# therealadityashankar/hey-buddy

Measured on AMD Instinct MI355X. Metric: audio clips/sec featurized+trained, 1.5 s @16 kHz, 1/2/4/8 GPU, higher is better.
Workload: dtype f32

## Files before the change

### hey-buddy_amd/csrc/hbk_augment.hip

```cpp
#include <algorithm>
#include <cmath>
#include <numeric>
#include <type_traits>
#include <vector>

#include "hbk_common.h"

namespace hbk {
namespace {

constexpr int kT = 23040;
constexpr int kM = kT / 2;
constexpr int kThreads = 1024;
constexpr int kN1 = 16000;
constexpr int kM1 = kN1 / 2;

template <bool INV>
__device__ __forceinline__ cf tw_const(double frac) {
  const double a = (INV ? 2.0 : -2.0) * M_PI * frac;
  return cf{static_cast<float>(cos(a)), static_cast<float>(sin(a))};
}

template <bool INV>
__device__ __forceinline__ void dft3(cf& a, cf& b, cf& c) {
// ... 1244 lines not shown
    tin[lc][32 + 4 * lq + 3] = p1.w;
    __syncthreads();
    const int tn = min(t0 + kEqTile, kT - kEqTile);
    p0 = *reinterpret_cast<const float4*>(xl + tn + 4 * lq);
    p1 = *reinterpret_cast<const float4*>(xl + tn + 32 + 4 * lq);
    for (int st0 = 0; st0 < kEqTile; st0 += 8) {
      const float4 ia = *reinterpret_cast<const float4*>(&tin[c][st0]);
      const float4 ib = *reinterpret_cast<const float4*>(&tin[c][st0 + 4]);
      const float in8[8] = {ia.x, ia.y, ia.z, ia.w, ib.x, ib.y, ib.z, ib.w};
      float o8[8];
#pragma unroll
      for (int q = 0; q < 8; ++q) {
        const float u = sec == 0 ? in8[q] : prev;
        const double vd = u;
        const double y = fma(b0, vd, s1);
        s1 = fma(b1, vd, fma(-a1, y, s2));
        s2 = fma(b2, vd, -a2 * y);
        const float v = static_cast<float>(y);
        o8[q] = v;
        prev = __builtin_bit_cast(float, __builtin_amdgcn_update_dpp(__builtin_bit_cast(int, prev),
                                                                     __builtin_bit_cast(int, v), 0x111, 0xF, 0xF,
                                                                     false));
      }
      if (sec == 6) {
        *reinterpret_cast<float4*>(&tout[c][st0]) = float4{o8[0], o8[1], o8[2], o8[3]};
        *reinterpret_cast<float4*>(&tout[c][st0 + 4]) = float4{o8[4], o8[5], o8[6], o8[7]};
      }
    }
    __syncthreads();
    if (store_l) {
#pragma unroll
      for (int m = 0; m < 8; ++m) {
        const int kk = lq + 8 * m;
        const int n = t0 - 6 + kk;
        if (n >= 0 && n < kT) ol[n] = tout[lc][kk];
      }
    }
    __syncthreads();
  }
}

constexpr int kPsFft = 250, kPsHop = 7, kPsBins = kPsFft / 2 + 1, kPsPad = kPsFft / 2;
constexpr int kPsTapMax = HBK_PITCH_SHIFT_MAX_TAPS;
constexpr int kPsPhaseMax = 128;
constexpr int kPsResFrames = 32;
#ifndef HBK_PV_ABLATE
#define HBK_PV_ABLATE 0
#endif
#ifndef HBK_PV_CLIPS
#define HBK_PV_CLIPS 2
#endif
constexpr int kPvClips = HBK_PV_CLIPS;
constexpr int kPvGroup = 8;
constexpr int kPvRows = 64;
constexpr int kPvGh = 64;
#ifndef HBK_PV_F32STATE
#define HBK_PV_F32STATE 0
#endif
#ifndef HBK_PV_RESTART
#if HBK_PV_F32STATE
#define HBK_PV_RESTART 128
#else
#define HBK_PV_RESTART 1024
#endif
#endif
constexpr int kPvRestart = HBK_PV_RESTART;
#if HBK_PV_F32STATE
typedef float pv_t;
#else
typedef double pv_t;
#endif

struct PitchArgs {
  const float* x;
  int64_t x_stride;
  const int32_t* idx;
  int n;
  float* out;
  int64_t out_stride;
  int L, f_in, f_out, l1, orig, nw, width, target;
  double rate;
  float* y;
  float* taps;
};

__device__ __forceinline__ int ps_i0(const PitchArgs& a, int t, float& alpha) {
  const float ts = static_cast<float>(static_cast<double>(t) * a.rate);
  const float fl = floorf(ts);
  alpha = ts - fl;
  return static_cast<int>(fl);
}

struct PvClip {
  float d[kPvRows][8];
  float xs[256];
  float gh[2][kPvGh][8];
  int cnt0;
};
struct PvShared {
  cf tw[256];
  double tw64[256][2];
  float4 wt[3][128];
  PvClip c[kPvClips];
};

__device__ __forceinline__ int pv_g(int b) { return (b & 3) ^ ((b & 4) ? 7 : 0); }

template <int kCtrl>
__device__ __forceinline__ float pv_dpp(float v) {
  return __builtin_bit_cast(float, __builtin_amdgcn_update_dpp(0, __builtin_bit_cast(int, v), kCtrl, 0xF, 0xF, true));
}

template <bool kSwap16>
__device__ __forceinline__ float pv_swap_add(float x, float y) {
  if (kSwap16)
    asm volatile("s_nop 1\n\tv_permlane16_swap_b32 %0, %1\n\ts_nop 1" : "+v"(x), "+v"(y));
  else
    asm volatile("s_nop 1\n\tv_permlane32_swap_b32 %0, %1\n\ts_nop 1" : "+v"(x), "+v"(y));
  return x + y;
}

__device__ __forceinline__ cf pv_cmul(cf a, cf b) {
  cf t, r;
  asm("v_pk_mul_f32 %0, %1, %2 op_sel_hi:[0,1]" : "=v"(t) : "v"(a), "v"(b));
  asm("v_pk_fma_f32 %0, %1, %2, %3 op_sel:[1,1,0] op_sel_hi:[1,0,1] neg_lo:[0,1,0]" : "=v"(r) : "v"(a), "v"(b), "v"(t));
  return r;
}
__device__ __forceinline__ cf pv_cmul_conj(cf a, cf b) {
  cf t, r;
  asm("v_pk_mul_f32 %0, %1, %2 op_sel_hi:[0,1] neg_hi:[0,1]" : "=v"(t) : "v"(a), "v"(b));
  asm("v_pk_fma_f32 %0, %1, %2, %3 op_sel:[1,1,0] op_sel_hi:[1,0,1]" : "=v"(r) : "v"(a), "v"(b), "v"(t));
  return r;
}

typedef float pv_v4 __attribute__((ext_vector_type(4)));
typedef __attribute__((address_space(3))) const pv_v4 pv_lds_v4;
__device__ __forceinline__ float4 pv_f4(pv_v4 v) { return float4{v.x, v.y, v.z, v.w}; }

__device__ __forceinline__ cf pv_inc(float4 da, float4 db, float4 w12, float4 w34, float4 w56) {
  const cf dxy = {da.x, da.y}, dzw = {da.z, da.w}, exy = {db.x, db.y}, ez = {db.z, db.w};
  const cf w1 = {w12.x, w12.y}, w2 = {w12.z, w12.w}, w3 = {w34.x, w34.y}, w4 = {w34.z, w34.w};
  const cf w5 = {w56.x, w56.y}, w6 = {w56.z, w56.w};
  cf acc;
  asm("v_pk_mul_f32 %0, %1, %2 op_sel:[1,0] op_sel_hi:[1,1]" : "=v"(acc) : "v"(dxy), "v"(w1));
  asm("v_pk_fma_f32 %0, %1, %2, %0 op_sel:[0,0,0] op_sel_hi:[0,1,1]" : "+v"(acc) : "v"(dzw), "v"(w2));
  asm("v_pk_fma_f32 %0, %1, %2, %0 op_sel:[1,0,0] op_sel_hi:[1,1,1]" : "+v"(acc) : "v"(dzw), "v"(w3));
  asm("v_pk_fma_f32 %0, %1, %2, %0 op_sel:[0,0,0] op_sel_hi:[0,1,1]" : "+v"(acc) : "v"(exy), "v"(w4));
  asm("v_pk_fma_f32 %0, %1, %2, %0 op_sel:[1,0,0] op_sel_hi:[1,1,1]" : "+v"(acc) : "v"(exy), "v"(w5));
  asm("v_pk_fma_f32 %0, %1, %2, %0 op_sel:[0,0,0] op_sel_hi:[0,1,1]" : "+v"(acc) : "v"(ez), "v"(w6));
  return acc;
}

__device__ __forceinline__ float ps_xp(const float* xr, int L, int p) {
  int i = p - kPsPad;
  i = i < 0 ? -i : i;
  i = i >= L ? 2 * (L - 1) - i : i;
  return xr[i];
}

__device__ __forceinline__ void pv_load_rows(const PitchArgs& a, PvShared& sh, const float* xr, int cl, int lane,
                                             int fb) {
  for (int q = lane; q < 2 * kPvRows; q += 128) {
    const int row = q >> 1, h = q & 1, f = fb + row;
    float* dr = sh.c[cl].d[row];
    if (f >= a.f_in) {
      for (int j = 4 * h; j < 4 * h + 4; ++j) dr[j] = 0.f;
      continue;
    }
    if (h == 0) {
      for (int j = 0; j < 4; ++j) dr[j] = ps_xp(xr, a.L, 7 * f + 243 + j) - ps_xp(xr, a.L, 7 * f - 7 + j);
    } else {
      int delta = 0;
      for (int j = 0; j < 7; ++j) {
        const float vin = ps_xp(xr, a.L, 7 * f + 243 + j), vout = ps_xp(xr, a.L, 7 * f - 7 + j);
        delta += (vin != 0.f) - (vout != 0.f);
        if (j >= 4) dr[j] = vin - vout;
      }
      dr[7] = __builtin_bit_cast(float, delta);
    }
  }
}

#ifdef HBK_PHASE_TIMING
#define HBK_PVT(i)                                     \
  do {                                                 \
    const unsigned long long t_ = __builtin_amdgcn_s_memtime(); \
    pvt[i] += t_ - pvt_t0;                             \
    pvt_t0 = t_;                                       \
  } while (0)
#else
#define HBK_PVT(i) \
  do {             \
  } while (0)
#endif

#ifndef HBK_PV_UNROLL_TAIL
#define HBK_PV_UNROLL_TAIL 1
#endif
#ifndef HBK_PV_WAVES
#define HBK_PV_WAVES 4
#endif
__global__ void __launch_bounds__(128 * kPvClips) __attribute__((amdgpu_waves_per_eu(HBK_PV_WAVES)))
ps_vocoder_kernel(PitchArgs a) {
#ifdef HBK_PHASE_TIMING
  unsigned long long pvt[5] = {0, 0, 0, 0, 0}, pvt_t0 = __builtin_amdgcn_s_memtime();
#endif
  extern __shared__ __attribute__((aligned(16))) unsigned char pv_smem[];
  PvShared& sh = *reinterpret_cast<PvShared*>(pv_smem);
  const int tid = threadIdx.x, cl = tid >> 7, lane = tid & 127;
  const int e = min(static_cast<int>(blockIdx.x) * kPvClips + cl, a.n - 1);
  const bool live = static_cast<int>(blockIdx.x) * kPvClips + cl < a.n;
  const float* xr = a.x + static_cast<int64_t>(a.idx[e]) * a.x_stride;
  PvClip& C = sh.c[cl];
  for (int q = tid; q < 256; q += blockDim.x) {
    double sn, cs;
    sincospi(2.0 * q / kPsFft, &sn, &cs);
    sh.tw[q] = cf{static_cast<float>(cs), static_cast<float>(sn)};
    sh.tw64[q][0] = cs;
    sh.tw64[q][1] = -sn;
  }
  if (lane == 0) C.cnt0 = 0;
  __syncthreads();
  int nz = 0;
  for (int q = lane; q < kPsFft; q += 128) {
    const float v = ps_xp(xr, a.L, q);
    C.xs[q] = v;
    nz += v != 0.f;
  }
  if (nz) atomicAdd(&C.cnt0, nz);
  for (int q = tid; q < 3 * 128; q += blockDim.x) {
    const int j = 2 * (q / 128) + 1, kk = min(q % 128, kPsBins - 1), q1 = (kk * j) % kPsFft,
              q2 = (kk * (j + 1)) % kPsFft;
    sh.wt[q / 128][q % 128] = float4{static_cast<float>(sh.tw64[q1][0]), static_cast<float>(sh.tw64[q1][1]),
                                     static_cast<float>(sh.tw64[q2][0]), static_cast<float>(sh.tw64[q2][1])};
  }
  int fb = 1;
  pv_load_rows(a, sh, xr, cl, lane, fb);
  __syncthreads();

  const int k = min(lane, kPsBins - 1);
  const int q7 = (7 * k) % kPsFft;
  const pv_t rr = static_cast<pv_t>(sh.tw64[q7][0]), ri = static_cast<pv_t>(-sh.tw64[q7][1]);
  const float ck = lane < kPsBins ? ((lane == 0 || lane == kPsBins - 1) ? 1.f : 2.f) : 0.f;
  const int gb = pv_g(lane & 7), w = lane >> 6, ou = (lane >> 3) & 7;
  cf esr[4], esi[4];
#pragma unroll
  for (int r = 0; r < 8; ++r) {
    const int sr = r ^ gb;
    const cf ev = sr < kPsHop ? ck * sh.tw[(k * sr) % kPsFft] : cf{0.f, 0.f};
    esr[r >> 1][r & 1] = ev.x;
    esi[r >> 1][r & 1] = -ev.y;
  }
  const bool b3 = lane & 8;
  auto direct = [&](double& re, double& im) {
    re = im = 0.0;
    int q = 0;
    for (int n = 0; n < kPsFft; ++n) {
      const double v = static_cast<double>(C.xs[n]);
      re = fma(v, sh.tw64[q][0], re);
      im = fma(v, sh.tw64[q][1], im);
      q += k;
      q -= q >= kPsFft ? kPsFft : 0;
    }
  };
  pv_t xre, xim;
  {
    double dre, dim;
    direct(dre, dim);
    xre = static_cast<pv_t>(dre);
    xim = static_cast<pv_t>(dim);
  }
  int cnt = __builtin_amdgcn_readfirstlane(C.cnt0);
  if (cnt == 0) xre = xim = pv_t(0);
  int sf = 0;
  int anchor = 0;
  static_assert(sizeof(sh.wt[0]) == 128 * sizeof(float4), "wt rows of 128 lanes");
  uint32_t wt_addr = static_cast<uint32_t>(reinterpret_cast<uintptr_t>((const pv_lds_v4*)&sh.wt[0][lane]));
  auto slide_to = [&](pv_t& nre, pv_t& nim, int& ncnt, const float* drow) {
    const int f = sf + 1;
    if (f >= a.f_in) {
      nre = nim = pv_t(0);
      ncnt = cnt;
      return;
    }
    asm volatile("" : "+v"(wt_addr));
    const pv_lds_v4* wtp = (const pv_lds_v4*)static_cast<uintptr_t>(wt_addr);
    const float4 w12 = pv_f4(wtp[0]), w34 = pv_f4(wtp[128]), w56 = pv_f4(wtp[256]);
    const float4* drv = reinterpret_cast<const float4*>(drow);
    const float4 da = drv[0], db = drv[1];
    cf acc = pv_inc(da, db, w12, w34, w56);
    acc.x += da.x;
    ncnt = cnt + __builtin_amdgcn_readfirstlane(__builtin_bit_cast(int, db.w));
    const pv_t ar = xre + static_cast<pv_t>(acc.x), ai = xim + static_cast<pv_t>(acc.y);
    nre = ar * rr - ai * ri;
    nim = ar * ri + ai * rr;
    if (ncnt == 0) nre = nim = pv_t(0);
  };
  auto commit = [&](pv_t nre, pv_t nim, int ncnt) {
    xre = nre;
    xim = nim;
    cnt = ncnt;
    ++sf;
  };
  auto polar_of = [&](pv_t re, pv_t im, cf& u, float& mag) {
    const float fr = static_cast<float>(re), fi = static_cast<float>(im);
    const float n2 = fmaf(fr, fr, fi * fi);
    const float rs = __builtin_amdgcn_rsqf(n2 + 0x1p-126f);
    u = cf{fr + 0x1p-63f, fi} * rs;
    mag = n2 * rs;
  };
  auto polar = [&](cf& u, float& mag) { polar_of(xre, xim, u, mag); };
  cf ca, na, pa;
  float cm, nm, pm;
  polar(ca, cm);
  {
    pv_t nre, nim;
    int ncnt;
    slide_to(nre, nim, ncnt, C.d[sf + 1 - fb]);
    commit(nre, nim, ncnt);
    polar(na, nm);
    slide_to(nre, nim, ncnt, C.d[sf + 1 - fb]);
    commit(nre, nim, ncnt);
    polar(pa, pm);
  }
  int c = 0;
  cf R = {1.f, 0.f};
  cf Q = {0.f, 0.f};
  int qz = 0;
  const int dq = q7;
  const cf e7 = sh.tw[q7];
  const int jmax = (a.l1 + kPsPad - 1) / kPsHop;
  float* y = a.y + static_cast<int64_t>(e) * a.l1;
  HBK_PVT(0);

  for (int t0 = 0; t0 <= jmax; t0 += kPvGroup) {
    {
      float al;
      const int tl = min(t0 + kPvGroup - 1, a.f_out - 1);
      const int need = t0 < a.f_out ? min(ps_i0(a, tl, al) + 3, a.f_in - 1) : 0;
      if (need >= fb + kPvRows) {
        __syncthreads();
        fb = sf + 1;
        pv_load_rows(a, sh, xr, cl, lane, fb);
        __syncthreads();
      }
    }
    if (sf - anchor >= kPvRestart && sf < a.f_in) {
      __syncthreads();
      for (int q = lane; q < kPsFft; q += 128) C.xs[q] = ps_xp(xr, a.L, kPsHop * sf + q);
      __syncthreads();
      double dre, dim;
      direct(dre, dim);
      xre = static_cast<pv_t>(dre);
      xim = static_cast<pv_t>(dim);
      if (cnt == 0) xre = xim = pv_t(0);
      anchor = sf;
    }
    HBK_PVT(1);
    R *= __builtin_amdgcn_rsqf(fmaf(R.x, R.x, R.y * R.y));
    cf tz = sh.tw[qz];
    const float* dg = C.d[0] + 8 * (sf + 1 - fb);
    float gr[kPvGroup];
    float al_lane = 0.f;
    int i0_lane = 0;
    auto frame = [&](int u, auto full) {
      constexpr bool FULL = decltype(full)::value;
      const int t = t0 + u;
#if HBK_PV_ABLATE & 2
      if (t < a.f_out) {
        float al;
        ps_i0(a, t, al);
        Q.x += al * tz.x;
      }
      if (false) {
#else
      if (FULL || t < a.f_out) {
#endif
        float al;
        int i0;
        if (FULL) {
          i0 = c + 1;
          al = __builtin_bit_cast(float, __builtin_amdgcn_readlane(__builtin_bit_cast(int, al_lane), u));
        } else {
          i0 = __builtin_amdgcn_readlane(i0_lane, u);
          al = __builtin_bit_cast(float, __builtin_amdgcn_readlane(__builtin_bit_cast(int, al_lane), u));
        }
        if (!FULL && i0 > c + 1) {
          ++c;
          ca = na;
          cm = nm;
          na = pa;
          nm = pm;
          R = cmul(R, cmul_conj(ca, na));
          pv_t nre, nim;
          int ncnt;
          slide_to(nre, nim, ncnt, C.d[sf + 1 - fb]);
          commit(nre, nim, ncnt);
          polar(pa, pm);
        }
        const bool step = FULL || i0 > c;
        if (!FULL && !step && t > 0) R = cmul(R, cmul_conj(na, ca));
        c += step ? 1 : 0;
        ca = step ? na : ca;
        cm = step ? nm : cm;
        na = step ? pa : na;
        nm = step ? pm : nm;
        pv_t nre, nim;
        int ncnt;
        slide_to(nre, nim, ncnt, FULL ? dg + 8 * u : C.d[sf + 1 - fb]);
        cf qa;
        float qm;
        polar_of(nre, nim, qa, qm);
        const float m = fmaf(al, nm - cm, cm);
        const cf P = pv_cmul(R, ca);
        const cf Z = pv_cmul_conj(P, tz);
        Q = __builtin_elementwise_fma(cf{m, m}, Z, Q);
        xre = step ? nre : xre;
        xim = step ? nim : xim;
        cnt = step ? ncnt : cnt;
        sf += step ? 1 : 0;
        pa = step ? qa : pa;
        pm = step ? qm : pm;
      }
      const cf vq = pv_cmul(Q, tz);
#if HBK_PV_ABLATE & 1
      gr[u] = vq.x * esr[u & 3].x;
#else
      cf pr[4];
#pragma unroll
      for (int j = 0; j < 4; ++j) pr[j] = __builtin_elementwise_fma(cf{vq.x, vq.x}, esr[j], cf{vq.y, vq.y} * esi[j]);
      const float q0 = pr[0].x + pv_dpp<0xB1>(pr[0].y), q1 = pr[1].x + pv_dpp<0xB1>(pr[1].y);
      const float q2 = pr[2].x + pv_dpp<0xB1>(pr[2].y), q3 = pr[3].x + pv_dpp<0xB1>(pr[3].y);
      const float h0 = q0 + pv_dpp<0x4E>(q1), h1 = q2 + pv_dpp<0x4E>(q3);
      const float gv = h0 + pv_dpp<0x141>(h1);
      if (FULL) {
        gr[u] = gv;
      } else {
#pragma unroll
        for (int j = 0; j < kPvGroup; ++j) gr[j] = j == u ? gv : gr[j];
      }
#endif
      tz = pv_cmul(tz, e7);
    };
    bool full = t0 + kPvGroup <= a.f_out;
    if (full) {
      float al;
      full = ps_i0(a, t0 + kPvGroup - 1, al) - c == kPvGroup;
    }
    i0_lane = ps_i0(a, t0 + (lane & 7), al_lane);
    if (full) {
#pragma unroll
      for (int u = 0; u < kPvGroup; ++u) frame(u, std::true_type{});
    } else {
#if HBK_PV_UNROLL_TAIL
#pragma unroll
#else
#pragma unroll 1
#endif
      for (int u = 0; u < kPvGroup; ++u) frame(u, std::false_type{});
    }
    qz = (qz + kPvGroup * dq) % kPsFft;
    float h[4];
#pragma unroll
    for (int i = 0; i < 4; ++i) {
      const float keep = b3 ? gr[2 * i + 1] : gr[2 * i], send = b3 ? gr[2 * i] : gr[2 * i + 1];
      h[i] = keep + pv_dpp<0x128>(send);
    }
    const float h02 = pv_swap_add<true>(h[0], h[1]), h13 = pv_swap_add<true>(h[2], h[3]);
    const float gsum = pv_swap_add<false>(h02, h13);
    HBK_PVT(2);
    if (gb < kPsHop) C.gh[w][(t0 + ou) % kPvGh][gb] = gsum;
    __syncthreads();
    HBK_PVT(3);
    if (lane < kPsHop * kPvGroup && live) {
      const int t = t0 + lane / kPsHop, r = lane % kPsHop;
      const int m = kPsHop * t + r - kPsPad;
      if (t <= jmax && m >= 0 && m < a.l1) {
        const float g1 = C.gh[0][t % kPvGh][r] + C.gh[1][t % kPvGh][r];
        float g2 = 0.f;
        if (r <= 4) {
          if (t >= 36) g2 = C.gh[0][(t - 36) % kPvGh][r + 2] + C.gh[1][(t - 36) % kPvGh][r + 2];
        } else if (t >= 35) {
          g2 = C.gh[0][(t - 35) % kPvGh][r - 5] + C.gh[1][(t - 35) % kPvGh][r - 5];
        }
        const int lo = max(0, t - 35 + (r >= 5 ? 1 : 0)), hi = min(a.f_out - 1, t);
        y[m] = (g1 - g2) * __builtin_amdgcn_rcpf(static_cast<float>(kPsFft) * static_cast<float>(hi - lo + 1));
      }
    }
    HBK_PVT(4);
  }
#ifdef HBK_PHASE_TIMING
  if (tid == 0)
    for (int i = 0; i < 5; ++i) atomicAdd(&g_aug_phase[16 + i], pvt[i]);
#endif
}

__global__ void ps_taps_kernel(PitchArgs a) {
  const int i = blockIdx.x * blockDim.x + threadIdx.x;
  if (i >= a.nw * kPsTapMax) return;
  const int ph = i / kPsTapMax, q = i % kPsTapMax;
  float v = 0.f;
  if (q < 2 * a.width + a.orig) {
    const double lpw = 6.0, base = min(a.orig, a.nw) * 0.99;
    double t = static_cast<double>(static_cast<float>(-ph) / static_cast<float>(a.nw)) +
               static_cast<double>(q - a.width) / a.orig;
    t = fmin(fmax(t * base, -lpw), lpw);
    const double c = cos(t * M_PI / lpw / 2);
    t *= M_PI;
    v = static_cast<float>((t == 0.0 ? 1.0 : sin(t) / t) * c * c * (base / a.orig));
  }
  a.taps[i] = v;
}

__global__ void __launch_bounds__(128) ps_resample_kernel(PitchArgs a) {
  static_assert(kPsTapMax % 2 == 0 && kPsResFrames % 2 == 0, "resampler pairs");
  constexpr int kPairs = kPsResFrames / 2;
  __shared__ __attribute__((aligned(16))) float ys2[kPairs][2 * kPsTapMax];
  const int ph = threadIdx.x, e = blockIdx.y;
  const int f0 = blockIdx.x * kPsResFrames;
  const float* y = a.y + static_cast<int64_t>(e) * a.l1;
  const int j0 = f0 * a.orig - a.width;
  for (int el = ph; el < kPsResFrames * kPsTapMax; el += 128) {
    const int fr = el / kPsTapMax, q = el - fr * kPsTapMax;
    const int src = j0 + fr * a.orig + q;
    ys2[fr >> 1][2 * q + (fr & 1)] = (src >= 0 && src < a.l1) ? y[src] : 0.f;
  }
  float tp[kPsTapMax];
  const float* tr = a.taps + min(ph, a.nw - 1) * kPsTapMax;
#pragma unroll
  for (int q = 0; q < kPsTapMax; ++q) tp[q] = tr[q];
  __syncthreads();
  if (ph >= a.nw) return;
  float* out = a.out + static_cast<int64_t>(a.idx[e]) * a.out_stride;
  for (int p = 0; p < kPairs; ++p) {
    const int i = (f0 + 2 * p) * a.nw + ph, i1 = i + a.nw;
    if (i >= a.L) break;
    cf v = {0.f, 0.f};
    if (i < a.target) {
      const float4* w = reinterpret_cast<const float4*>(ys2[p]);
#pragma unroll
      for (int q2 = 0; q2 < kPsTapMax / 2; ++q2) {
        const float4 ww = w[q2];
        v = __builtin_elementwise_fma(cf{tp[2 * q2], tp[2 * q2]}, cf{ww.x, ww.y}, v);
        v = __builtin_elementwise_fma(cf{tp[2 * q2 + 1], tp[2 * q2 + 1]}, cf{ww.z, ww.w}, v);
      }
    }
    out[i] = v.x;
    if (i1 < a.L) out[i1] = i1 < a.target ? v.y : 0.f;
  }
}


constexpr int kRsFrames = 64, kRsK = 160, kRsLd = kRsK + 8;
static_assert(kPsTapMax <= kRsK && kPsPhaseMax <= 128, "the MFMA resampler's K padding and 8 phase tiles");
typedef _Float16 rs_h8 __attribute__((ext_vector_type(8)));
typedef float rs_f4 __attribute__((ext_vector_type(4)));
__device__ __forceinline__ void rs_split(float v, _Float16& h, _Float16& l) {
  h = static_cast<_Float16>(v);
  l = static_cast<_Float16>(v - static_cast<float>(h));
}
__global__ void __launch_bounds__(256) ps_resample_mfma_kernel(PitchArgs a) {
  __shared__ __attribute__((aligned(16))) _Float16 wh[kRsFrames][kRsLd];
  __shared__ __attribute__((aligned(16))) _Float16 wl[kRsFrames][kRsLd];
  __shared__ float red[4];
  const int tid = threadIdx.x, lane = tid & 63, wave = tid >> 6;
  const int e = blockIdx.y, f0 = blockIdx.x * kRsFrames;
  const float* y = a.y + static_cast<int64_t>(e) * a.l1;
  constexpr int kPairs = kRsFrames * kRsK / 2, kPer = kPairs / 256;
  float v0[kPer], v1[kPer];
  float mx = 0.f;
#pragma unroll
  for (int u = 0; u < kPer; ++u) {
    const int p = tid + 256 * u, fr = p / (kRsK / 2), q = 2 * (p - fr * (kRsK / 2));
    const int src = (f0 + fr) * a.orig - a.width + q;
    const int s0 = min(max(src, 0), a.l1 - 1), s1 = min(max(src + 1, 0), a.l1 - 1);
    const float x0 = y[s0], x1 = y[s1];
    v0[u] = (src >= 0 && src < a.l1 && q < kPsTapMax) ? x0 : 0.f;
    v1[u] = (src + 1 >= 0 && src + 1 < a.l1 && q + 1 < kPsTapMax) ? x1 : 0.f;
    mx = fmaxf(mx, fmaxf(fabsf(v0[u]), fabsf(v1[u])));
  }
  const int n = lane & 15, kq = lane >> 4;
  rs_h8 bh[2][5], bl[2][5];
#pragma unroll
  for (int t = 0; t < 2; ++t) {
    const int ph = min(16 * (2 * wave + t) + n, a.nw - 1);
    const float* tr = a.taps + ph * kPsTapMax;
#pragma unroll
    for (int ks = 0; ks < 5; ++ks)
#pragma unroll
      for (int j = 0; j < 8; ++j) {
        const int q = 32 * ks + 8 * kq + j;
        const float tv = tr[min(q, kPsTapMax - 1)];
        _Float16 h, l;
        rs_split(q < kPsTapMax ? tv * 1024.f : 0.f, h, l);
        bh[t][ks][j] = h;
        bl[t][ks][j] = l;
      }
  }
  for (int o = 32; o >= 1; o >>= 1) mx = fmaxf(mx, __shfl_xor(mx, o, 64));
  if (lane == 0) red[wave] = mx;
  __syncthreads();
  mx = fmaxf(fmaxf(red[0], red[1]), fmaxf(red[2], red[3]));
  const int ex = mx > 0.f ? min(14 - ilogbf(mx), 100) : 0;
  const float scale = ldexpf(1.f, ex), unscale = ldexpf(1.f, -ex - 10);
#pragma unroll
  for (int u = 0; u < kPer; ++u) {
    const int p = tid + 256 * u, fr = p / (kRsK / 2), q = 2 * (p - fr * (kRsK / 2));
    _Float16 h0, l0, h1, l1;
    rs_split(v0[u] * scale, h0, l0);
    rs_split(v1[u] * scale, h1, l1);
    wh[fr][q] = h0;
    wh[fr][q + 1] = h1;
    wl[fr][q] = l0;
    wl[fr][q + 1] = l1;
  }
  __syncthreads();
  float* out = a.out + static_cast<int64_t>(a.idx[e]) * a.out_stride;
#pragma unroll
  for (int ft = 0; ft < kRsFrames / 16; ++ft) {
    rs_f4 acc[2] = {{0.f, 0.f, 0.f, 0.f}, {0.f, 0.f, 0.f, 0.f}};
#pragma unroll
    for (int ks = 0; ks < 5; ++ks) {
      const rs_h8 ah = *reinterpret_cast<const rs_h8*>(&wh[16 * ft + n][32 * ks + 8 * kq]);
      const rs_h8 al = *reinterpret_cast<const rs_h8*>(&wl[16 * ft + n][32 * ks + 8 * kq]);
#pragma unroll
      for (int t = 0; t < 2; ++t) {
        acc[t] = __builtin_amdgcn_mfma_f32_16x16x32_f16(ah, bh[t][ks], acc[t], 0, 0, 0);
        acc[t] = __builtin_amdgcn_mfma_f32_16x16x32_f16(ah, bl[t][ks], acc[t], 0, 0, 0);
        acc[t] = __builtin_amdgcn_mfma_f32_16x16x32_f16(al, bh[t][ks], acc[t], 0, 0, 0);
      }
    }
#pragma unroll
    for (int t = 0; t < 2; ++t) {
      const int ph = 16 * (2 * wave + t) + n;
#pragma unroll
      for (int j = 0; j < 4; ++j) {
        const int i = (f0 + 16 * ft + 4 * kq + j) * a.nw + ph;
        if (ph < a.nw && i < a.L) out[i] = i < a.target ? acc[t][j] * unscale : 0.f;
      }
    }
  }
}

}
}

struct hbk_reverb_plan {
  float2* thi = nullptr;
  float2* tlo = nullptr;
  float2* twn = nullptr;
  float2* thi8 = nullptr;
  float2* tlo8 = nullptr;
  float2* twn16 = nullptr;
};

namespace {
constexpr size_t kAugLds = (size_t(2 * hbk::kM + 32) * sizeof(float)) + (hbk::kTwHi + hbk::kTwLo) * sizeof(float2);
constexpr size_t kBandStopLds = kAugLds + (5 * hbk::kBsCirc + 1) * sizeof(float);
constexpr size_t kColoredLds = (size_t(2 * hbk::kM1 + 32) * sizeof(float)) + (hbk::kTw8Hi + hbk::kTw8Lo) * sizeof(float2);
}

// ... 369 lines not shown

int hbk_tanh_distortion(const float* x, int64_t n_clips, int64_t x_stride, const float* amount,
                        const int32_t* idx, int64_t n_entries, float* out, int64_t out_stride, void* stream) {
  using namespace hbk;
  if (n_clips < 0) return arg_error("negative n_clips");
  if (n_clips == 0) return HBK_OK;
  if (!x || !out || !amount) return arg_error("NULL pointer");
  if (x_stride < kT || out_stride < kT) return arg_error("stride < 23040");
  TanhArgs a;
  a.x = x;
  a.x_stride = x_stride;
  a.out = out;
  a.out_stride = out_stride;
  a.n_clips = n_clips;
  a.amount = amount;
  a.idx = idx;
  a.n_entries = idx ? n_entries : n_clips;
  if (a.n_entries <= 0) return n_entries < 0 ? arg_error("negative n_entries") : HBK_OK;
  const int64_t blocks = std::min<int64_t>(a.n_entries, persistent_blocks(2, stream));
  hipLaunchKernelGGL(tanh_distortion_kernel, dim3(unsigned(blocks)), dim3(kThreads), 0, as_stream(stream), a);
  HBK_LAUNCH_CHECK("tanh_distortion_kernel");
  return HBK_OK;
}

int hbk_seven_band_eq(const float* x, int64_t n_clips, int64_t x_stride, const double* coef, const int32_t* idx,
                      int64_t n_entries, float* out, int64_t out_stride, void* stream) {
  using namespace hbk;
  if (n_clips < 0 || n_entries < 0) return arg_error("negative count");
  if (!idx) n_entries = n_clips;
  if (n_entries == 0) return HBK_OK;
  if (!x || !out || !coef) return arg_error("NULL pointer");
  if (x_stride < kT || out_stride < kT) return arg_error("stride < 23040");
  if ((reinterpret_cast<uintptr_t>(x) | reinterpret_cast<uintptr_t>(out)) % 16 || x_stride % 4 || out_stride % 4)
    return arg_error("x / out rows must be 16-B aligned");
  EqArgs a;
  a.x = x;
  a.x_stride = x_stride;
  a.coef = coef;
  a.idx = idx;
  a.out = out;
  a.out_stride = out_stride;
  a.n = n_entries;
  hipLaunchKernelGGL(eq_kernel, dim3(unsigned((n_entries + kEqClips - 1) / kEqClips)), dim3(64), 0,
                     as_stream(stream), a);
  HBK_LAUNCH_CHECK("eq_kernel");
  return HBK_OK;
}

static int ps_geometry(int64_t L, int32_t sample_rate, int32_t num, int32_t den, hbk::PitchArgs& a) {
  using namespace hbk;
  if (sample_rate != 16000) {
    set_error("hbk: pitch shift supports 16 kHz (n_fft 250, hop 7), got %d", sample_rate);
    return HBK_ERR_UNSUPPORTED;
  }
  if (num <= 0 || den <= 0) return arg_error("shift num / den must be positive");
  if (L <= kPsPad || L > (int64_t(1) << 24)) return arg_error("clip length must be in (125, 2^24]");
  a.L = static_cast<int>(L);
  a.rate = double(den) / double(num);
  a.f_in = 1 + a.L / kPsHop;
  a.f_out = static_cast<int>(std::ceil(double(a.f_in) / a.rate));
  a.l1 = kPsHop * (a.f_out - 1);
  const int64_t new_sr = int64_t(sample_rate) * den / num;
  const int64_t g = std::gcd(int64_t(sample_rate), new_sr);
  if (new_sr <= 0 || g <= 0) return arg_error("shift out of range");
  a.orig = static_cast<int>(sample_rate / g);
  a.nw = static_cast<int>(new_sr / g);
  a.width = static_cast<int>(std::ceil(6.0 * a.orig / (std::min(a.orig, a.nw) * 0.99)));
  a.target = static_cast<int>(std::ceil(double(a.nw) * a.l1 / a.orig));
  if (a.nw > kPsPhaseMax || 2 * a.width + a.orig > kPsTapMax || a.l1 <= 0 ||
      a.rate * kPvGroup + 3 > kPvRows) {
    set_error("hbk: pitch shift %d/%d resamples %d -> %d (%d taps): the kernel holds <= %d phases of <= %d taps "
              "(torch_pitch_shift's fast shifts at 16 kHz)", num, den, a.orig, a.nw, 2 * a.width + a.orig,
              kPsPhaseMax, kPsTapMax);
    return HBK_ERR_UNSUPPORTED;
  }
  return HBK_OK;
}

static int64_t ps_bytes(const hbk::PitchArgs& a, int64_t n, int64_t* off) {
  using namespace hbk;
  auto up = [](int64_t b) { return (b + 255) & ~int64_t(255); };
  off[0] = off[1] = off[2] = off[3] = 0;
  off[4] = up(n * a.l1 * 4);
  return off[4] + up(int64_t(kPsPhaseMax) * kPsTapMax * 4);
}

int64_t hbk_pitch_shift_workspace_size(int64_t n, int64_t T, int32_t sample_rate, int32_t num, int32_t den) {
  hbk::PitchArgs a{};
  if (n <= 0 || ps_geometry(T, sample_rate, num, den, a) != HBK_OK) return 0;
  int64_t off[5];
  return ps_bytes(a, n, off);
}

int hbk_pitch_shift(const float* x, int64_t x_stride, int64_t n, const int32_t* idx, int64_t T, int32_t sample_rate,
                    int32_t num, int32_t den, float* out, int64_t out_stride, void* workspace,
                    int64_t workspace_bytes, void* stream) {
  using namespace hbk;
  if (n < 0) return arg_error("negative n");
  if (n == 0) return HBK_OK;
  if (n > 65535) return arg_error("n > 65535 per call");
  if (!x || !idx || !out || !workspace) return arg_error("NULL pointer");
  PitchArgs a{};
  const int rc = ps_geometry(T, sample_rate, num, den, a);
  if (rc != HBK_OK) return rc;
  if (x_stride < T || out_stride < T) return arg_error("stride < T");
  int64_t off[5];
  if (workspace_bytes < ps_bytes(a, n, off)) return arg_error("workspace too small (hbk_pitch_shift_workspace_size)");
  unsigned char* w = static_cast<unsigned char*>(workspace);
  a.x = x;
  a.x_stride = x_stride;
  a.idx = idx;
  a.out = out;
  a.out_stride = out_stride;
  a.n = static_cast<int>(n);
  a.y = reinterpret_cast<float*>(w + off[3]);
  a.taps = reinterpret_cast<float*>(w + off[4]);
  hipStream_t st = as_stream(stream);
  hipLaunchKernelGGL(ps_taps_kernel, dim3(unsigned((a.nw * kPsTapMax + 255) / 256)), dim3(256), 0, st, a);
  HBK_LAUNCH_CHECK("ps_taps_kernel");
  static bool lds_set = false;
  if (!lds_set) {
    HBK_HIP(hipFuncSetAttribute(reinterpret_cast<const void*>(ps_vocoder_kernel),
                                hipFuncAttributeMaxDynamicSharedMemorySize, int(sizeof(PvShared))));
    lds_set = true;
  }
  hipLaunchKernelGGL(ps_vocoder_kernel, dim3(unsigned((n + kPvClips - 1) / kPvClips)), dim3(128 * kPvClips),
                     sizeof(PvShared), st, a);
  HBK_LAUNCH_CHECK("ps_vocoder_kernel");
  const int res_frames = (a.L + a.nw - 1) / a.nw;
  static const bool valu_rs = getenv("HBK_PS_RESAMPLE_VALU") != nullptr;
  if (valu_rs || a.nw > 128) {
    hipLaunchKernelGGL(ps_resample_kernel, dim3(unsigned((res_frames + kPsResFrames - 1) / kPsResFrames), unsigned(n)),
                       dim3(128), 0, st, a);
    HBK_LAUNCH_CHECK("ps_resample_kernel");
  } else {
    hipLaunchKernelGGL(ps_resample_mfma_kernel, dim3(unsigned((res_frames + kRsFrames - 1) / kRsFrames), unsigned(n)),
                       dim3(256), 0, st, a);
    HBK_LAUNCH_CHECK("ps_resample_mfma_kernel");
  }
  return HBK_OK;
}

}

#ifdef HBK_PHASE_TIMING
extern "C" int hbk_debug_aug_phase(unsigned long long* out) {
  if (hipMemcpyFromSymbol(out, HIP_SYMBOL(hbk::g_aug_phase), sizeof(unsigned long long) * 32) != hipSuccess)
    return -2;
  unsigned long long z[32] = {};
  (void)hipMemcpyToSymbol(HIP_SYMBOL(hbk::g_aug_phase), z, sizeof(z));
  return 0;
}
#endif
```

### hey-buddy_amd/heybuddy/util/numpy_util.py

```python
from __future__ import annotations

import os
import struct
import threading
from typing import Any, Optional, Tuple

import numpy as np

__all__ = ["AppendableNumpyArrayFile", "read_npy_header", "load_to_device"]

_MAGIC = b"\x93NUMPY"
_RESERVE = 21
_ALIGN = 64


def _render_header(rows: int, tail: Tuple[int, ...], descr: str, size: Optional[int] = None) -> bytes:
    shape = (rows, *tail)
    body = "{'descr': %r, 'fortran_order': False, 'shape': %r, }" % (descr, shape)
    body += " " * (_RESERVE - len(str(rows)))
    fixed = len(_MAGIC) + 4
    need = fixed + len(body) + 1
    if size is None:
        size = (need + _ALIGN - 1) // _ALIGN * _ALIGN
    elif need > size:
# ... 49 lines not shown
            raise ValueError(f"{self.filename}: object dtype cannot be appended to")
        if self.dtype is not None and self.dtype != dtype:
            raise ValueError(f"{self.filename} stores {dtype}; {self.dtype} was requested")
        if not shape:
            raise ValueError(f"{self.filename}: a 0-d array has no axis to grow")
        _render_header(shape[0], shape[1:], np.lib.format.dtype_to_descr(dtype), offset)
        size = os.path.getsize(self.filename)
        expect = offset + int(np.prod(shape)) * dtype.itemsize
        if size != expect:
            raise ValueError(f"{self.filename} holds {size - offset} data bytes but its header says "
                             f"{expect - offset}: the file needs recovery before appending")
        self.dtype, self.shape, self.header_length, self._end = dtype, shape, offset, size
        self._fd = os.open(self.filename, os.O_RDWR)

    def _header(self) -> bytes:
        return _render_header(self.shape[0], self.shape[1:], np.lib.format.dtype_to_descr(self.dtype),
                              self.header_length)

    def update_header(self) -> None:
        with self.lock:
            if self._fd is not None:
                os.pwrite(self._fd, self._header(), 0)

    def append(self, arr: np.ndarray) -> None:
        arr = np.asarray(arr)
        if arr.ndim == 0:
            raise ValueError("cannot append a 0-d array")
        with self.lock:
            if self._fd is None:
                self.dtype = self.dtype or arr.dtype
                self.shape = (0, *arr.shape[1:])
                self._fd = os.open(self.filename, os.O_RDWR | os.O_CREAT | os.O_TRUNC, 0o644)
                self.header_length = len(_render_header(0, self.shape[1:], np.lib.format.dtype_to_descr(self.dtype)))
                self._end = self.header_length
                os.pwrite(self._fd, self._header(), 0)
            if tuple(arr.shape[1:]) != tuple(self.shape[1:]):
                raise ValueError(f"cannot append rows of shape {arr.shape[1:]} to {self.filename}, "
                                 f"whose rows are {self.shape[1:]}")
            data = np.ascontiguousarray(arr, dtype=self.dtype)
            if data.nbytes:
                _pwrite_all(self._fd, data.reshape(-1).view(np.uint8), self._end)
            self._end += data.nbytes
            self.shape = (self.shape[0] + arr.shape[0], *self.shape[1:])
            if self.rewrite_header_on_append:
                os.pwrite(self._fd, self._header(), 0)

    def close(self) -> None:
        with self.lock:
            if self._fd is None:
                return
            os.pwrite(self._fd, self._header(), 0)
            os.close(self._fd)
            self._fd = None

    def __del__(self) -> None:
        try:
            self.close()
        except Exception:
            pass

    def __enter__(self) -> "AppendableNumpyArrayFile":
        return self

    def __exit__(self, *exc) -> None:
        self.close()


def load_to_device(path: str, device, dtype=None, chunk_rows: int = 65536, rows: Optional[slice] = None):
    import torch

    mm = np.load(path, mmap_mode="r")
    if rows is not None:
        mm = mm[rows]
    src_dtype = torch.from_numpy(np.empty(0, dtype=mm.dtype)).dtype
    out = torch.empty(mm.shape, dtype=dtype or src_dtype, device=device)
    if mm.shape[0] == 0:
        return out
    n = min(chunk_rows, mm.shape[0])
    pinned = torch.empty((n, *mm.shape[1:]), dtype=src_dtype).pin_memory() if torch.cuda.is_available() \
        else torch.empty((n, *mm.shape[1:]), dtype=src_dtype)
    stage = torch.empty((n, *mm.shape[1:]), dtype=src_dtype, device=device)
    for r0 in range(0, mm.shape[0], n):
        k = min(n, mm.shape[0] - r0)
        if torch.cuda.is_available():
            torch.cuda.current_stream(out.device).synchronize()
        pinned[:k].numpy()[...] = mm[r0:r0 + k]
        stage[:k].copy_(pinned[:k], non_blocking=True)
        out[r0:r0 + k].copy_(stage[:k])
    return out
```

Measured before the change: 933,500.

## Skip silent regions in phase-vocoder pitch shift and resampler

Each clip is scanned for the first and last non-zero sample. The vocoder loop then runs only over the output frames that can be non-zero, writes zeros where every contributing frame is silent, and records the valid y range per clip. The resample kernels use that range to return early and write zeros for windows that fall entirely in silence. This cuts vocoder and resample work on zero-padded clips, at the cost of an extra scan over each clip and some more complex restart logic that could drift from the full computation.

After: 950,500 (median of 6 runs). 1.02x the previous value.

```diff
diff --git a/hey-buddy_amd/csrc/hbk_augment.hip b/hey-buddy_amd/csrc/hbk_augment.hip
--- a/hey-buddy_amd/csrc/hbk_augment.hip
+++ b/hey-buddy_amd/csrc/hbk_augment.hip
@@ -1350,6 +1350,8 @@
   double rate;
   float* y;
   float* taps;
+  int2* yr;
+  int span;
 };
 
 __device__ __forceinline__ int ps_i0(const PitchArgs& a, int t, float& alpha) {
@@ -1364,6 +1366,7 @@
   float xs[256];
   float gh[2][kPvGh][8];
   int cnt0;
+  int lo, hi;
 };
 struct PvShared {
   cf tw[256];
@@ -1446,6 +1449,43 @@
       }
       dr[7] = __builtin_bit_cast(float, delta);
     }
+  }
+}
+
+__device__ __forceinline__ void pv_scan_span(PvClip& C, const float* xr, int L, int lane) {
+  int lo = INT_MAX, hi = -1;
+  int done = 0;
+  if ((reinterpret_cast<uintptr_t>(xr) & 15) == 0) {
+    const float4* x4 = reinterpret_cast<const float4*>(xr);
+    const int n4 = L >> 2;
+    for (int q0 = 0; q0 < n4; q0 += 128 * 8) {
+      float4 v[8];
+#pragma unroll
+      for (int j = 0; j < 8; ++j) {
+        const int q = q0 + 128 * j + lane;
+        v[j] = q < n4 ? x4[q] : float4{0.f, 0.f, 0.f, 0.f};
+      }
+#pragma unroll
+      for (int j = 0; j < 8; ++j) {
+        const int p = 4 * (q0 + 128 * j + lane);
+        const bool b0 = v[j].x != 0.f, b1 = v[j].y != 0.f, b2 = v[j].z != 0.f, b3 = v[j].w != 0.f;
+        if (b0 || b1 || b2 || b3) {
+          lo = min(lo, p + (b0 ? 0 : b1 ? 1 : b2 ? 2 : 3));
+          hi = max(hi, p + (b3 ? 3 : b2 ? 2 : b1 ? 1 : 0));
+        }
+      }
+    }
+    done = 4 * n4;
+  }
+  for (int p = done + lane; p < L; p += 128) {
+    if (xr[p] != 0.f) {
+      lo = min(lo, p);
+      hi = max(hi, p);
+    }
+  }
+  if (hi >= 0) {
+    atomicMin(&C.lo, lo);
+    atomicMax(&C.hi, hi);
   }
 }
 
@@ -1488,7 +1528,12 @@
     sh.tw64[q][1] = -sn;
   }
   if (lane == 0) C.cnt0 = 0;
+  if (lane == 0) {
+    C.lo = INT_MAX;
+    C.hi = -1;
+  }
   __syncthreads();
+  if (a.span) pv_scan_span(C, xr, a.L, lane);
   int nz = 0;
   for (int q = lane; q < kPsFft; q += 128) {
     const float v = ps_xp(xr, a.L, q);
@@ -1531,15 +1576,14 @@
       q -= q >= kPsFft ? kPsFft : 0;
     }
   };
-  pv_t xre, xim;
-  {
+  pv_t xre = pv_t(0), xim = pv_t(0);
+  int cnt = __builtin_amdgcn_readfirstlane(C.cnt0);
+  if (cnt != 0) {
     double dre, dim;
     direct(dre, dim);
     xre = static_cast<pv_t>(dre);
     xim = static_cast<pv_t>(dim);
   }
-  int cnt = __builtin_amdgcn_readfirstlane(C.cnt0);
-  if (cnt == 0) xre = xim = pv_t(0);
   int sf = 0;
   int anchor = 0;
   static_assert(sizeof(sh.wt[0]) == 128 * sizeof(float4), "wt rows of 128 lanes");
@@ -1581,11 +1625,13 @@
   cf ca, na, pa;
   float cm, nm, pm;
   polar(ca, cm);
+  int cntc = cnt, cntn, lastnz = INT_MIN / 2;
   {
     pv_t nre, nim;
     int ncnt;
     slide_to(nre, nim, ncnt, C.d[sf + 1 - fb]);
     commit(nre, nim, ncnt);
+    cntn = cnt;
     polar(na, nm);
     slide_to(nre, nim, ncnt, C.d[sf + 1 - fb]);
     commit(nre, nim, ncnt);
@@ -1599,9 +1645,67 @@
   const cf e7 = sh.tw[q7];
   const int jmax = (a.l1 + kPsPad - 1) / kPsHop;
   float* y = a.y + static_cast<int64_t>(e) * a.l1;
+  auto frames_of = [&](int lo, int hi, int& tb, int& tl) {
+    tb = 0;
+    tl = jmax;
+    float al;
+    if (lo > hi) {
+      tl = -1;
+      return;
+    }
+    if (lo > 2 * kPsPad && a.rate < 2.0) {
+      const int fz = (lo - kPsPad) / kPsHop - 1;
+      int tg = min(static_cast<int>((fz - 2) / a.rate), a.f_out - 1) & ~(kPvGroup - 1);
+      while (tg > 0 && ps_i0(a, tg - 1, al) + 2 > fz) tg -= kPvGroup;
+      tb = max(tg, 0);
+    }
+    if (hi < a.L - 1 - 2 * kPsPad) {
+      const int fn = min((hi + kPsPad) / kPsHop, a.f_in - 1);
+      int t = max(min(a.f_out - 1, static_cast<int>((fn + 1) / a.rate) + 1), 0);
+      while (t > 0 && ps_i0(a, t, al) > fn) --t;
+      while (t + 1 < a.f_out && ps_i0(a, t + 1, al) <= fn) ++t;
+      tl = min(jmax, t + 36);
+    }
+  };
+  int t_beg = 0, t_last = jmax;
+  {
+    int tb = 0, tl = jmax;
+    if (a.span) {
+      int lo = INT_MAX, hi = -1;
+      for (int i = 0; i < kPvClips; ++i) {
+        lo = min(lo, sh.c[i].lo);
+        hi = max(hi, sh.c[i].hi);
+      }
+      frames_of(lo, hi, t_beg, t_last);
+      frames_of(C.lo, C.hi, tb, tl);
+    }
+    if (lane == 0 && live)
+      a.yr[e] = tl < tb ? int2{0, 0}
+                        : int2{max(kPsHop * tb - kPsPad, 0), min(kPsHop * (tl + 1) - kPsPad, a.l1)};
+  }
+  if (t_beg > 0) {
+    for (int t0 = kPvGroup; t0 < t_beg; t0 += kPvGroup) {
+      float al;
+      const int s = ps_i0(a, t0 - 1, al) + 2;
+      if (s - anchor >= kPvRestart && s < a.f_in) anchor = s;
+    }
+    float al;
+    c = ps_i0(a, t_beg - 1, al);
+    sf = c + 2;
+    xre = xim = pv_t(0);
+    cnt = cntc = cntn = 0;
+    ca = na = pa = cf{1.f, 0.f};
+    cm = nm = pm = 0.f;
+    qz = ((t_beg % kPsFft) * dq) % kPsFft;
+    __syncthreads();
+    for (int q = lane; q < 2 * kPvGh * 8; q += 128) (&C.gh[0][0][0])[q] = 0.f;
+    fb = sf + 1;
+    pv_load_rows(a, sh, xr, cl, lane, fb);
+    __syncthreads();
+  }
   HBK_PVT(0);
 
-  for (int t0 = 0; t0 <= jmax; t0 += kPvGroup) {
+  for (int t0 = t_beg; t0 <= t_last; t0 += kPvGroup) {
     {
       float al;
       const int tl = min(t0 + kPvGroup - 1, a.f_out - 1);
@@ -1617,17 +1721,20 @@
       __syncthreads();
       for (int q = lane; q < kPsFft; q += 128) C.xs[q] = ps_xp(xr, a.L, kPsHop * sf + q);
       __syncthreads();
-      double dre, dim;
-      direct(dre, dim);
-      xre = static_cast<pv_t>(dre);
-      xim = static_cast<pv_t>(dim);
-      if (cnt == 0) xre = xim = pv_t(0);
+      xre = xim = pv_t(0);
+      if (cnt != 0) {
+        double dre, dim;
+        direct(dre, dim);
+        xre = static_cast<pv_t>(dre);
+        xim = static_cast<pv_t>(dim);
+      }
       anchor = sf;
     }
     HBK_PVT(1);
     R *= __builtin_amdgcn_rsqf(fmaf(R.x, R.x, R.y * R.y));
     cf tz = sh.tw[qz];
     const float* dg = C.d[0] + 8 * (sf + 1 - fb);
+    int gor = 0;
     float gr[kPvGroup];
     float al_lane = 0.f;
     int i0_lane = 0;
@@ -1655,6 +1762,8 @@
         }
         if (!FULL && i0 > c + 1) {
           ++c;
+          cntc = cntn;
+          cntn = cnt;
           ca = na;
           cm = nm;
           na = pa;
@@ -1669,6 +1778,9 @@
         const bool step = FULL || i0 > c;
         if (!FULL && !step && t > 0) R = cmul(R, cmul_conj(na, ca));
         c += step ? 1 : 0;
+        cntc = step ? cntn : cntc;
+        cntn = step ? cnt : cntn;
+        gor |= cntc | cntn;
         ca = step ? na : ca;
         cm = step ? nm : cm;
         na = step ? pa : na;
@@ -1752,9 +1864,11 @@
           g2 = C.gh[0][(t - 35) % kPvGh][r - 5] + C.gh[1][(t - 35) % kPvGh][r - 5];
         }
         const int lo = max(0, t - 35 + (r >= 5 ? 1 : 0)), hi = min(a.f_out - 1, t);
-        y[m] = (g1 - g2) * __builtin_amdgcn_rcpf(static_cast<float>(kPsFft) * static_cast<float>(hi - lo + 1));
-      }
-    }
+        const float v = (g1 - g2) * __builtin_amdgcn_rcpf(static_cast<float>(kPsFft) * static_cast<float>(hi - lo + 1));
+        y[m] = (gor == 0 && t - lastnz > 35) ? 0.f : v;
+      }
+    }
+    if (gor) lastnz = t0 + kPvGroup - 1;
     HBK_PVT(4);
   }
 #ifdef HBK_PHASE_TIMING
@@ -1780,6 +1894,15 @@
   a.taps[i] = v;
 }
 
+__device__ __forceinline__ bool ps_window_silent(const PitchArgs& a, int2 yr, int e, int j0, int f0, int frames,
+                                                 int tid, int threads) {
+  if (j0 < yr.y && j0 + (frames - 1) * a.orig + kPsTapMax > yr.x) return false;
+  float* out = a.out + static_cast<int64_t>(a.idx[e]) * a.out_stride;
+  const int i1 = static_cast<int>(min(static_cast<int64_t>(f0 + frames) * a.nw, static_cast<int64_t>(a.L)));
+  for (int i = f0 * a.nw + tid; i < i1; i += threads) out[i] = 0.f;
+  return true;
+}
+
 __global__ void __launch_bounds__(128) ps_resample_kernel(PitchArgs a) {
   static_assert(kPsTapMax % 2 == 0 && kPsResFrames % 2 == 0, "resampler pairs");
   constexpr int kPairs = kPsResFrames / 2;
@@ -1788,10 +1911,12 @@
   const int f0 = blockIdx.x * kPsResFrames;
   const float* y = a.y + static_cast<int64_t>(e) * a.l1;
   const int j0 = f0 * a.orig - a.width;
+  const int2 yr = a.yr[e];
+  if (ps_window_silent(a, yr, e, j0, f0, kPsResFrames, ph, 128)) return;
   for (int el = ph; el < kPsResFrames * kPsTapMax; el += 128) {
     const int fr = el / kPsTapMax, q = el - fr * kPsTapMax;
     const int src = j0 + fr * a.orig + q;
-    ys2[fr >> 1][2 * q + (fr & 1)] = (src >= 0 && src < a.l1) ? y[src] : 0.f;
+    ys2[fr >> 1][2 * q + (fr & 1)] = (src >= yr.x && src < yr.y) ? y[src] : 0.f;
   }
   float tp[kPsTapMax];
   const float* tr = a.taps + min(ph, a.nw - 1) * kPsTapMax;
@@ -1834,6 +1959,8 @@
   const int tid = threadIdx.x, lane = tid & 63, wave = tid >> 6;
   const int e = blockIdx.y, f0 = blockIdx.x * kRsFrames;
   const float* y = a.y + static_cast<int64_t>(e) * a.l1;
+  const int2 yr = a.yr[e];
+  if (ps_window_silent(a, yr, e, f0 * a.orig - a.width, f0, kRsFrames, tid, 256)) return;
   constexpr int kPairs = kRsFrames * kRsK / 2, kPer = kPairs / 256;
   float v0[kPer], v1[kPer];
   float mx = 0.f;
@@ -1843,8 +1970,8 @@
     const int src = (f0 + fr) * a.orig - a.width + q;
     const int s0 = min(max(src, 0), a.l1 - 1), s1 = min(max(src + 1, 0), a.l1 - 1);
     const float x0 = y[s0], x1 = y[s1];
-    v0[u] = (src >= 0 && src < a.l1 && q < kPsTapMax) ? x0 : 0.f;
-    v1[u] = (src + 1 >= 0 && src + 1 < a.l1 && q + 1 < kPsTapMax) ? x1 : 0.f;
+    v0[u] = (src >= yr.x && src < yr.y && q < kPsTapMax) ? x0 : 0.f;
+    v1[u] = (src + 1 >= yr.x && src + 1 < yr.y && q + 1 < kPsTapMax) ? x1 : 0.f;
     mx = fmaxf(mx, fmaxf(fabsf(v0[u]), fabsf(v1[u])));
   }
   const int n = lane & 15, kq = lane >> 4;
@@ -2380,13 +2507,14 @@
   auto up = [](int64_t b) { return (b + 255) & ~int64_t(255); };
   off[0] = off[1] = off[2] = off[3] = 0;
   off[4] = up(n * a.l1 * 4);
-  return off[4] + up(int64_t(kPsPhaseMax) * kPsTapMax * 4);
+  off[5] = off[4] + up(int64_t(kPsPhaseMax) * kPsTapMax * 4);
+  return off[5] + up(n * int64_t(sizeof(int2)));
 }
 
 int64_t hbk_pitch_shift_workspace_size(int64_t n, int64_t T, int32_t sample_rate, int32_t num, int32_t den) {
   hbk::PitchArgs a{};
   if (n <= 0 || ps_geometry(T, sample_rate, num, den, a) != HBK_OK) return 0;
-  int64_t off[5];
+  int64_t off[6];
   return ps_bytes(a, n, off);
 }
 
@@ -2402,7 +2530,7 @@
   const int rc = ps_geometry(T, sample_rate, num, den, a);
   if (rc != HBK_OK) return rc;
   if (x_stride < T || out_stride < T) return arg_error("stride < T");
-  int64_t off[5];
+  int64_t off[6];
   if (workspace_bytes < ps_bytes(a, n, off)) return arg_error("workspace too small (hbk_pitch_shift_workspace_size)");
   unsigned char* w = static_cast<unsigned char*>(workspace);
   a.x = x;
@@ -2413,6 +2541,12 @@
   a.n = static_cast<int>(n);
   a.y = reinterpret_cast<float*>(w + off[3]);
   a.taps = reinterpret_cast<float*>(w + off[4]);
+  a.yr = reinterpret_cast<int2*>(w + off[5]);
+  static const bool span_off = [] {
+    const char* s = getenv("HBK_PS_SPAN");
+    return s && s[0] == '0';
+  }();
+  a.span = span_off ? 0 : 1;
   hipStream_t st = as_stream(stream);
   hipLaunchKernelGGL(ps_taps_kernel, dim3(unsigned((a.nw * kPsTapMax + 255) / 256)), dim3(256), 0, st, a);
   HBK_LAUNCH_CHECK("ps_taps_kernel");
diff --git a/hey-buddy_amd/heybuddy/util/numpy_util.py b/hey-buddy_amd/heybuddy/util/numpy_util.py
--- a/hey-buddy_amd/heybuddy/util/numpy_util.py
+++ b/hey-buddy_amd/heybuddy/util/numpy_util.py
@@ -155,7 +155,7 @@
     stage = torch.empty((n, *mm.shape[1:]), dtype=src_dtype, device=device)
     for r0 in range(0, mm.shape[0], n):
         k = min(n, mm.shape[0] - r0)
-        if torch.cuda.is_available():
+        if out.is_cuda:
             torch.cuda.current_stream(out.device).synchronize()
         pinned[:k].numpy()[...] = mm[r0:r0 + k]
         stage[:k].copy_(pinned[:k], non_blocking=True)
```
